# NVlabs/DREAM

Measured on AMD Instinct MI355X. Metric: frames/s DREAM-vgg-q 400x400 b=128 inference, higher is better.
Workload: dtype f32

## Files before the change

dream_amd/csrc/conv_wino4.hip:

```cpp
#include <type_traits>
#include <stdlib.h>
#include <dream_cdna4.h>
#include "common.h"
#include "pack_device.h"
#include "../../include/dream_hip.h"

#ifndef DREAM_W4_DIAG
#define DREAM_W4_DIAG 0
#endif
#ifndef DREAM_W4_STORE
#define DREAM_W4_STORE buffer_store_f32
#endif
#ifndef DREAM_W4_MIDBARRIER
#define DREAM_W4_MIDBARRIER 0
#endif
#ifndef DREAM_W4_STAGGER_N
#define DREAM_W4_STAGGER_N 0
#define DREAM_W4_STAGGER_PCT 0
#endif
#ifndef DREAM_W4_WAUX
#define DREAM_W4_WAUX 0
#endif
#ifndef DREAM_W4_XAUX
#define DREAM_W4_XAUX 0
#endif
#ifndef DREAM_W4_STAG_LX
#define DREAM_W4_STAG_LX 0
#endif
#ifndef DREAM_W4_RUNNING_WOFF
#define DREAM_W4_RUNNING_WOFF 1
#endif
#ifndef DREAM_W4_SETPRIO
#define DREAM_W4_SETPRIO 0
#endif

namespace {

struct Wino4Params {
    const float *x;
    const float *u;
    const float *scale;
    const float *shift;
    const float *residual;
    float *y;
    float *y_full;
    int B, H, W, Cin, Cout, CoutPad;
    int TY, TX;
    int ntiles;
    int nblk, blk_per_xcd;
    unsigned long long magic_tpi, magic_tx;
    int flags;
    int out_scale, out_oy, out_ox;
    int in_scale, in_oy, in_ox;
    int stagger_n, stagger_unit;
    int ymap;
};

constexpr int W4T = 16;
constexpr int W4P = 36;
#ifndef DREAM_W4_RING
#define DREAM_W4_RING 8
#endif
#ifndef DREAM_W4_NARROW_RING
#define DREAM_W4_NARROW_RING 18
#endif
#ifndef DREAM_W4_PAT_RING
#define DREAM_W4_PAT_RING 10
#endif
#ifndef DREAM_W4_PAT_S1OFF
#define DREAM_W4_PAT_S1OFF 8
#endif


template <bool NARROW>
struct W4Cfg {
    static constexpr int NW = NARROW ? 4 : 8;
    static constexpr int K = NARROW ? 8 : 16;
    static constexpr int Q = K / 4;
    static constexpr int KS = K / 4;
    static constexpr int PAD = 16 * NW;
    static constexpr int VPS = NARROW ? W4T * K : W4T * K + 16;
    static constexpr int VB = W4P * VPS;
    static constexpr int SROW = NARROW ? 14 : 25;
    static constexpr int QS = NARROW ? 7 : 6;
    static constexpr int SB = W4T * 6 * SROW * 4;
    static constexpr int RING = NARROW ? DREAM_W4_NARROW_RING : DREAM_W4_RING;
    static constexpr int AHEAD = RING - 2;
    static_assert(72 % RING == 0, "the weight ring must divide two chunks' positions");
    using vec = std::conditional_t<NARROW, f32x2, f32x4>;
};
template <bool NARROW>
DREAM_DEVICE int v4_slot(int q, int t) { return NARROW ? q ^ ((t >> 3) & 1) : q ^ ((t >> 2) & 2); }

DREAM_DEVICE f32x4 fma4(float c, f32x4 a, f32x4 b) {
    f32x4 r;
#pragma unroll
    for (int k = 0; k < 4; ++k) r[k] = __builtin_fmaf(c, a[k], b[k]);
    return r;
}

DREAM_DEVICE f32x4 sub4(f32x4 y, f32x4 x) { return pk_sub4(y, x); }
DREAM_DEVICE f32x4 bt_row(int j, const f32x4 *d) {
    switch (j) {
        case 0: return fma4(-2.0f, d[2], fma4(1.5f, sub4(d[3], d[1]), d[0] + d[4]));
        case 1: return fma4(2.5f, d[3], fma4(0.5f, d[2], sub4(d[4], d[1])));
        case 2: return fma4(0.5f, d[3], fma4(-2.5f, d[2], d[4] + d[1]));
        case 3: return fma4(2.0f, sub4(d[3], d[1]), sub4(d[4], d[2]));
        case 4: return fma4(-0.5f, sub4(d[3], d[1]), sub4(d[4], d[2]));
        default: return fma4(-2.0f, d[3], fma4(1.5f, sub4(d[4], d[2]), d[1] + d[5]));
    }
}

DREAM_DEVICE constexpr bool pat4_row_active(int pat, int i) { return pat == 0 || (((pat - 1) >> 1) == 0 ? i <= 4 : i >= 1); }
DREAM_DEVICE constexpr bool pat4_col_active(int pat, int j) { return pat == 0 || (((pat - 1) & 1) == 0 ? j <= 4 : j >= 1); }
DREAM_DEVICE constexpr bool pat4_active(int pat, int pp) { return pat4_row_active(pat, pp / 6) && pat4_col_active(pat, pp % 6); }
DREAM_DEVICE constexpr int pat4_count(int pat) { return pat == 0 ? 36 : 25; }
struct Pat4Table { int pos[36]; };
constexpr Pat4Table pat4_table(int pat) {
    Pat4Table t = {};
    int n = 0;
    for (int pp = 0; pp < 36; ++pp)
        if (pat4_active(pat, pp)) t.pos[n++] = pp;
    return t;
}
template <int PAT>
struct Pat4 { static constexpr Pat4Table table = pat4_table(PAT); };
#define pat4_pos(PAT, k) (Pat4<PAT>::table.pos[k])

template <int MODE, bool NARROW, int PAT = 0>
__global__ void __launch_bounds__(64 * W4Cfg<NARROW>::NW, 2) conv_wino4_kernel(const Wino4Params p) {
    using C = W4Cfg<NARROW>;
    using vec = typename C::vec;
    constexpr int W4K = C::K, W4NW = C::NW, V4PS = C::VPS, V4B = C::VB, S4ROW = C::SROW;
    constexpr int NPOS = pat4_count(PAT);
    constexpr int W4_RING = PAT ? DREAM_W4_PAT_RING : C::RING, W4_AHEAD = W4_RING - 2;
    static_assert((2 * NPOS) % W4_RING == 0, "the weight ring must divide two chunks' positions");
    DREAM_DYNAMIC_LDS(float, sV);
    const int tid = threadIdx.x;
    const int lane = tid & 63;
    const int wave = wave_index();
    const int item_id = wave * 48 + (lane < 48 ? lane : lane - 16);

    const int xcd = (int)(blockIdx.x & 7), J = (int)(gridDim.x >> 3);
    const int part = p.ymap ? xcd / p.ymap : xcd;
    const int blk_hi = (part + 1) * p.blk_per_xcd;
    const int blk_end = blk_hi < p.nblk ? blk_hi : p.nblk;
    int tb = part * p.blk_per_xcd + (int)(blockIdx.x >> 3);
    if (tb >= blk_end) return;
    const int n0 = (p.ymap ? xcd % p.ymap : (int)blockIdx.y) * (16 * W4NW);
    if (p.stagger_n > 1) {
        const unsigned w = blockIdx.x + blockIdx.y * gridDim.x;
        const int naps = (int)((w * 2654435761u >> 16) % (unsigned)p.stagger_n) * p.stagger_unit;
        for (int i = 0; i < naps; ++i) __builtin_amdgcn_s_sleep(127);
    }
    const int tiles_per_img = p.TY * p.TX;
    const int Si = PAT ? p.in_scale : 1;
    const size_t img_floats = (size_t)(Si * p.H) * (Si * p.W) * p.Cin;

    const int q1 = item_id % C::Q, r1 = (item_id / C::Q) % 6, t1 = (item_id / C::Q) / 6;
    const int s1_off = ((t1 * 6 + r1) * S4ROW + C::QS * q1) * 4;
    const int q2 = item_id % C::Q;
    const int j2 = NARROW ? (item_id >> 3) % 6 : (item_id >> 2) % 6;
    const int t2 = NARROW ? 4 * (item_id / 48) + ((item_id >> 1) & 3) : (item_id >> 2) / 6;
    const int s2_off = ((t2 * 6) * S4ROW + C::QS * q2 + j2) * 4;
    const int v2_off = j2 * V4PS + t2 * W4K + 4 * v4_slot<NARROW>(q2, t2);

    unsigned goff0;
    int item1 = t1 | (r1 << 8) | (q1 << 16);
    auto plan_item = [&](int tile0, int b0) {
        asm volatile("" : "+v"(item1));
        const int t = item1 & 255, r = (item1 >> 8) & 255, q = (item1 >> 16) & 255;
        const int tau = tile0 + t;
        const bool tv = tau < p.ntiles;
        const int b = div_magic40(tau, p.magic_tpi), rem = tau - b * tiles_per_img;
        const int ty = div_magic40(rem, p.magic_tx), tx = rem - ty * p.TX;
        const int gy = 4 * ty - 1 + r, x0 = 4 * tx - 1;
        const bool rok = tv & ((unsigned)gy < (unsigned)p.H);
        goff0 = PAT ? (unsigned)(((((b - b0) * Si * p.H + Si * gy + p.in_oy) * (Si * p.W) + Si * x0 + p.in_ox) * p.Cin + 4 * q) * 4)
                    : (unsigned)(((((b - b0) * p.H + gy) * p.W + x0) * p.Cin + 4 * q) * 4);
        item1 &= 0xffffff;
#pragma unroll
        for (int c = 0; c < 6; ++c) item1 |= (rok & ((unsigned)(x0 + c) < (unsigned)p.W)) ? (1 << (24 + c)) : 0;
    };
    const unsigned px_in = (unsigned)(Si * p.Cin * 4);
    auto item_offset = [&](int c) {
        if (DREAM_W4_DIAG & 16) {
            unsigned o = BUFFER_OOB;
            asm volatile("" : "+v"(o));
            return o;
        }
        return (item1 >> (24 + c)) & 1 ? goff0 + (unsigned)c * px_in : BUFFER_OOB;
    };
    auto block_tile0 = [&](int blk) { return blk < blk_end ? blk * W4T : p.ntiles; };
    auto block_xbuf = [&](int b0) {
        return make_buffer(p.x + (size_t)b0 * img_floats, ((size_t)(p.B - b0) * img_floats) * sizeof(float));
    };

    const int lt = lane & 15, lg = lane >> 4;
    const int a_off = NARROW ? lt * W4K + 4 * v4_slot<NARROW>(lg >> 1, lt) + 2 * (lg & 1) : lt * W4K + 4 * v4_slot<NARROW>(lg, lt);
    const unsigned b_lane = (unsigned)(((wave * 16 + lt) * W4K + C::KS * lg) * 4);
    const unsigned u_pos_stride = (unsigned)(p.CoutPad * W4K * 4);
    const BufferRsrc ubuf = make_buffer(p.u + (size_t)n0 * W4K, ((size_t)((p.Cin / W4K) * W4P + C::AHEAD) * p.CoutPad - (size_t)n0) * W4K * sizeof(float));

    f32x4 acc[W4P];
    const int nchunks = p.Cin / W4K;
    if (DREAM_W4_SETPRIO && wave >= W4NW / 2) __builtin_amdgcn_s_setprio(1);

    vec bq[W4_RING];
    auto load_u = [&](unsigned soff) {
        if constexpr (NARROW) return buffer_load_x2(ubuf, b_lane, soff);
        else return buffer_load_x4_aux<DREAM_W4_WAUX>(ubuf, b_lane, soff);
    };
#pragma unroll
    for (int k = 0; k < W4_AHEAD; ++k) bq[k] = load_u((unsigned)pat4_pos(PAT, k) * u_pos_stride);
    unsigned woff = (unsigned)W4_AHEAD * u_pos_stride;
    DREAM_OPAQUE_SGPR(woff);

    f32x4 *const sV4 = (f32x4 *)sV;
    vec *const sVa = (vec *)sV;
    int vrd[2], vwr[2], s1p = (2 * V4B + s1_off) / 4, s2p = (2 * V4B + s2_off) / 4;
#pragma unroll
    for (int h = 0; h < 2; ++h) {
        vrd[h] = (h * V4B + a_off) / C::KS;
        vwr[h] = (h * V4B + v2_off) / 4;
        asm volatile("" : "+v"(vrd[h]), "+v"(vwr[h]));
    }
    asm volatile("" : "+v"(s1p), "+v"(s2p));
    f32x4 d[6];
    auto pass1_piece = [&](int j) { sV4[s1p + j] = bt_row(j, d); };
    auto pass2_read = [&](int r) { d[r] = sV4[s2p + r * S4ROW]; };
    auto pass2_piece = [&](int i, int h) { if (pat4_row_active(PAT, i)) sV4[vwr[h] + i * (6 * V4PS / 4)] = bt_row(i, d); };

    vec a[2][2];
    auto read_a = [&](int set, int k, int h) {
        const int p0 = pat4_pos(PAT, k), p1 = pat4_pos(PAT, k + 1 < NPOS ? k + 1 : k);
        if constexpr (NARROW) {
            a[set][0] = lds_read_unmerged(sVa + vrd[h] + p0 * V4PS / C::KS);
            a[set][1] = lds_read_unmerged(sVa + vrd[h] + p1 * V4PS / C::KS);
        } else {
            a[set][0] = sVa[vrd[h] + p0 * V4PS / C::KS];
            if (k + 1 < NPOS) a[set][1] = sVa[vrd[h] + p1 * V4PS / C::KS];
        }
    };

    int tile0 = block_tile0(tb);
    int b0 = div_magic40(tile0, p.magic_tpi);
    BufferRsrc xbuf = block_xbuf(b0);
    plan_item(tile0, b0);
#pragma unroll
    for (int c = 0; c < 6; ++c) d[c] = buffer_load_x4(xbuf, item_offset(c), 0u);
#pragma unroll
    for (int j = 0; j < 6; ++j) pass1_piece(j);
    __syncthreads();
#pragma unroll
    for (int r = 0; r < 6; ++r) pass2_read(r);
#pragma unroll
    for (int i = 0; i < 6; ++i) pass2_piece(i, 0);
    __syncthreads();

    auto chunk = [&](auto ph_tag, auto stag_tag, bool last, int c, int tile0n, int b0n) __attribute__((always_inline)) {
        constexpr int PH = decltype(ph_tag)::value;
        constexpr int STAG = decltype(stag_tag)::value;
#ifndef DREAM_W4_S1
#define DREAM_W4_S1 10
#define DREAM_W4_S2 13
#define DREAM_W4_LX 3
#endif
        constexpr int NSLOT = (NPOS + 1) / 2;
        constexpr int S1 = PAT ? NSLOT - DREAM_W4_PAT_S1OFF : DREAM_W4_S1, S2 = PAT ? S1 + 3 : DREAM_W4_S2;
        constexpr int LX = PAT ? 1 : DREAM_W4_LX;
        constexpr int LX0 = STAG ? DREAM_W4_STAG_LX : 0;
        static_assert(LX0 + LX <= S1, "the patch loads must be issued before pass 1");
        const unsigned coff = last ? 0u : (unsigned)((c + 1) * W4K * 4);
        const int cnext = last ? 0 : (c + 1) * W4P;
        if (PH == 1 && last) xbuf = block_xbuf(b0n);
        read_a(0, 0, PH);
        __builtin_amdgcn_sched_barrier(0);
#pragma unroll
        for (int s = 0; s < NSLOT; ++s) {
            const int k0 = 2 * s;
            const bool two = k0 + 1 < NPOS;
            const int pp = pat4_pos(PAT, k0), pp1 = pat4_pos(PAT, two ? k0 + 1 : k0);
            auto load_b = [&](int half) {
                if ((DREAM_W4_DIAG & 2) || (half && !two)) return;
                const int kn = k0 + half + W4_AHEAD;
                if constexpr (PAT == 0 && DREAM_W4_RUNNING_WOFF && !(DREAM_W4_DIAG & 32)) {
                    if (kn == NPOS && last) woff = 0u;
                    bq[(PH * NPOS + kn) % W4_RING] = load_u(woff);
                    woff += u_pos_stride;
                    DREAM_OPAQUE_SGPR(woff);
                } else {
                    const int spos = kn >= NPOS ? cnext + pat4_pos(PAT, kn - NPOS) : c * W4P + pat4_pos(PAT, kn);
                    bq[(PH * NPOS + kn) % W4_RING] = load_u((DREAM_W4_DIAG & 32) ? 0u : (unsigned)spos * u_pos_stride);
                }
            };
            auto load_x = [&](int col) { if (!(DREAM_W4_DIAG & 1)) d[col] = buffer_load_x4_aux<DREAM_W4_XAUX>(xbuf, item_offset(col), (DREAM_W4_DIAG & 64) ? 0u : coff); };
            auto pair = [&](int r) {
                const int i0 = (PH * NPOS + k0) % W4_RING, i1 = (PH * NPOS + k0 + 1) % W4_RING;
                acc[pp] = mfma_f32_16x16x4(a[s & 1][0][r], bq[i0][r], acc[pp]);
                if (two) acc[pp1] = mfma_f32_16x16x4(a[s & 1][1][r], bq[i1][r], acc[pp1]);
                __builtin_amdgcn_sched_barrier(0);
            };
            auto after = [&](int k) {
                if (k == 0) {
                    load_b(0);
                    if (s + 1 < NSLOT) read_a((s + 1) & 1, k0 + 2, PH);
                    if (PH == 1 && s == 0 && last) plan_item(tile0n, b0n);
                    if (s >= LX0 && s < LX0 + LX) { for (int c2 = 0; c2 < 3 / LX; ++c2) load_x((6 / LX) * (s - LX0) + c2); }
                    if (!(DREAM_W4_DIAG & 8) && s >= S1 && s < S1 + 3) pass1_piece(2 * (s - S1));
                    if (!(DREAM_W4_DIAG & 8) && s == S2) { pass2_read(0); pass2_read(1); }
                    if (!(DREAM_W4_DIAG & 8) && s > S2 && s <= S2 + 3) pass2_piece(2 * (s - S2 - 1), 1 - PH);
                } else if (k == 1) {
                    load_b(1);
                    if (s >= LX0 && s < LX0 + LX) { for (int c2 = 3 / LX; c2 < 6 / LX; ++c2) load_x((6 / LX) * (s - LX0) + c2); }
                    if (!(DREAM_W4_DIAG & 8) && s == S2) { pass2_read(2); pass2_read(3); }
                } else if (k == 2) {
                    if (!(DREAM_W4_DIAG & 8) && s >= S1 && s < S1 + 3) pass1_piece(2 * (s - S1) + 1);
                    if (!(DREAM_W4_DIAG & 8) && s == S2) { pass2_read(4); pass2_read(5); }
                    if (!(DREAM_W4_DIAG & 8) && s > S2 && s <= S2 + 3) pass2_piece(2 * (s - S2 - 1) + 1, 1 - PH);
                }
            };
            if constexpr (NARROW) {
                pair(0);
                after(0);
                after(1);
                pair(1);
                after(2);
            } else {
                pair(0);
                after(0);
                pair(1);
                after(1);
                pair(2);
                after(2);
                pair(3);
            }
            if (s == S1 + 2 && !(DREAM_W4_DIAG & 4)) {
                if (DREAM_W4_MIDBARRIER) __syncthreads();
                __builtin_amdgcn_sched_barrier(0);
            }
        }
        if (!(DREAM_W4_DIAG & 4)) __syncthreads();
    };
    const std::integral_constant<int, 0> ph0{};
    const std::integral_constant<int, 1> ph1{};

    constexpr bool pool = MODE == 1 || MODE == 4, both = MODE == 4, has_res = MODE == 2 || MODE == 3, mask = MODE == 3;
    auto epilogue = [&](auto site_tag, int tile0e, int b0e) {
        if (DREAM_W4_DIAG & 128) {
#pragma unroll
            for (int pp = 0; pp < W4P; ++pp)
                if (pat4_active(PAT, pp)) asm volatile("" :: "v"(acc[pp]));
            return;
        }
        const auto &e = *DREAM_KERNARG_SITE(p, decltype(site_tag)::value);
        const bool relu = (e.flags & DREAM_CONV_RELU) != 0;
        const bool late = MODE == 2 && (e.flags & DREAM_CONV_RES_AFTER_RELU) != 0;
        const int Ho = pool ? e.H / 2 : e.H, Wo = pool ? e.W / 2 : e.W, So = e.out_scale;
        const size_t out_img = (size_t)(So * Ho) * (So * Wo) * e.Cout;
        const unsigned px_b = (unsigned)(So * e.Cout * 4), row_b = (unsigned)(So * So * Wo * e.Cout * 4);
        const int ln = lane_id();
        const int lt = ln & 15, lg = ln >> 4;
        const int col = n0 + wave * 16 + lt;
        const bool cok = col < e.Cout;
        const float sc = (e.scale != nullptr && cok) ? e.scale[col] : 1.0f;
        const float sh = (e.shift != nullptr && cok) ? e.shift[col] : 0.0f;
        const BufferRsrc ybuf = make_buffer(e.y + (size_t)b0e * out_img, (DREAM_W4_DIAG & 256) ? 0 : (size_t)(e.B - b0e) * out_img * sizeof(float));
        const BufferRsrc rbuf = make_buffer(has_res ? e.residual + (size_t)b0e * out_img : e.y,
                                            has_res ? (size_t)(e.B - b0e) * out_img * sizeof(float) : 0);
        const size_t full_img = (size_t)e.H * e.W * e.Cout;
        const unsigned fpx_b = (unsigned)(e.Cout * 4), frow_b = (unsigned)(e.W * e.Cout * 4);
        const BufferRsrc fbuf = make_buffer(both ? e.y_full + (size_t)b0e * full_img : e.y, both ? (size_t)(e.B - b0e) * full_img * sizeof(float) : 0);
        const int tau0 = tile0e + lg * 4;
        int b = div_magic40(tau0, p.magic_tpi);
        const int rem = tau0 - b * tiles_per_img;
        int ty = div_magic40(rem, p.magic_tx), tx = rem - ty * p.TX;
        constexpr int NS = pool ? 2 : 4;
        unsigned basef[2][2];
        int limf[2][2];
        unsigned base4[2][2];
        int lim4[2][2];
        constexpr int FULL = pool ? 0x33 : 0xff;
#pragma unroll
        for (int rp = 0; rp < 2; ++rp)
#pragma unroll
            for (int h = 0; h < 2; ++h) {
                const bool tok = cok & ((tau0 + 2 * rp + h) < p.ntiles);
                const int oy = NS * ty, ox = NS * tx;
                base4[rp][h] = (unsigned)(((((b - b0e) * So * Ho + So * oy + e.out_oy) * (So * Wo) + So * ox + e.out_ox) * e.Cout + col) * 4);
                int m = 0;
#pragma unroll
                for (int i = 0; i < NS; ++i) m |= ((oy + i) < Ho ? 1 << i : 0) | ((ox + i) < Wo ? 16 << i : 0);
                lim4[rp][h] = tok ? m : 0;
                if (both) {
                    basef[rp][h] = (unsigned)(((((b - b0e) * e.H + 4 * ty) * e.W + 4 * tx) * e.Cout + col) * 4);
                    int mf = 0;
#pragma unroll
                    for (int i = 0; i < 4; ++i) mf |= ((4 * ty + i) < e.H ? 1 << i : 0) | ((4 * tx + i) < e.W ? 16 << i : 0);
                    limf[rp][h] = tok ? mf : 0;
                }
                const bool wrap_x = (tx + 1 == p.TX);
                const bool wrap_y = wrap_x & (ty + 1 == p.TY);
                tx = wrap_x ? 0 : tx + 1;
                ty = wrap_y ? 0 : (wrap_x ? ty + 1 : ty);
                b += wrap_y ? 1 : 0;
            }
        auto out_off4 = [&](int rp, int h, int i, int jj) {
            const bool inb = ((lim4[rp][h] >> i) & (lim4[rp][h] >> (4 + jj)) & 1) != 0;
            return inb ? base4[rp][h] + (unsigned)i * row_b + (unsigned)jj * px_b : BUFFER_OOB;
        };
        bool interior4[2];
#pragma unroll
        for (int rp = 0; rp < 2; ++rp) interior4[rp] = wave_all((lim4[rp][0] == FULL) & (lim4[rp][1] == FULL));
        auto load_col0 = [&](int rp, float (&r)[2][4]) {
            if (interior4[rp]) {
#pragma unroll
                for (int h = 0; h < 2; ++h)
#pragma unroll
                    for (int i = 0; i < 4; ++i) r[h][i] = buffer_load_f32(rbuf, base4[rp][h], (unsigned)i * row_b);
            } else {
#pragma unroll
                for (int h = 0; h < 2; ++h)
#pragma unroll
                    for (int i = 0; i < 4; ++i) r[h][i] = buffer_load_f32(rbuf, out_off4(rp, h, i, 0), 0u);
            }
        };
        float r0[2][4], r0n[2][4];
        if (has_res) load_col0(0, r0);
#pragma unroll
        for (int rp = 0; rp < 2; ++rp) {
            const unsigned (&base)[2] = base4[rp];
            auto out_off = [&](int h, int i, int jj) { return out_off4(rp, h, i, jj); };
            const bool all_interior = interior4[rp];
            auto fm = [](float c, f32x2 x, f32x2 y) { return __builtin_elementwise_fma(f32x2{c, c}, x, y); };
            f32x2 sA[6][4];
#pragma unroll
            for (int i = 0; i < 6; ++i) {
                f32x2 m[6];
#pragma unroll
                for (int j = 0; j < 6; ++j)
                    m[j] = pat4_active(PAT, 6 * i + j) ? f32x2{acc[6 * i + j][2 * rp], acc[6 * i + j][2 * rp + 1]} : f32x2{0.0f, 0.0f};
                const f32x2 t1 = pk_sub2(m[1], m[2]), t2 = m[1] + m[2];
                sA[i][0] = (m[0] + t2) + (m[3] + m[4]);
                sA[i][1] = fm(-2.0f, m[4], fm(0.5f, m[3], t1));
                sA[i][2] = fm(4.0f, m[4], fm(0.25f, m[3], t2));
                sA[i][3] = fm(-8.0f, m[4], fm(0.125f, m[3], t1)) + m[5];
            }
            auto finish = [&](float v, float rv) {
                if (has_res) v = mask ? (rv > 0.0f ? v : 0.0f) : (late ? v : v + rv);
                const float vr = fmaxf(v, 0.0f);
                v = relu ? vr : v;
                return (MODE == 2 && late) ? v + rv : v;
            };
            auto columns = [&](auto interior_tag, auto &rcur) {
                constexpr bool interior = decltype(interior_tag)::value;
                auto voff = [&](int h, int i, int j2) { return interior ? base[h] : out_off(h, i, j2); };
                auto soff = [&](int i, int j2) { return interior ? (unsigned)i * row_b + (unsigned)j2 * px_b : 0u; };
                float keep[2][2];
#pragma unroll
                for (int jj = 0; jj < 4; ++jj) {
                    float rnext[2][4];
                    if (has_res && jj == 3 && rp == 0) load_col0(1, r0n);
                    if (has_res && jj + 1 < 4) {
#pragma unroll
                        for (int h = 0; h < 2; ++h)
#pragma unroll
                            for (int i = 0; i < 4; ++i) rnext[h][i] = buffer_load_f32(rbuf, voff(h, i, jj + 1), soff(i, jj + 1));
                    }
                    const f32x2 t1 = pk_sub2(sA[1][jj], sA[2][jj]), t2 = sA[1][jj] + sA[2][jj];
                    f32x2 o4[4];
                    o4[0] = (sA[0][jj] + t2) + (sA[3][jj] + sA[4][jj]);
                    o4[1] = fm(-2.0f, sA[4][jj], fm(0.5f, sA[3][jj], t1));
                    o4[2] = fm(4.0f, sA[4][jj], fm(0.25f, sA[3][jj], t2));
                    o4[3] = fm(-8.0f, sA[4][jj], fm(0.125f, sA[3][jj], t1)) + sA[5][jj];
#pragma unroll
                    for (int i = 0; i < 4; ++i) o4[i] = o4[i] * f32x2{sc, sc} + f32x2{sh, sh};
#pragma unroll
                    for (int h = 0; h < 2; ++h) {
                        if (pool) {
                            float v[4];
#pragma unroll
                            for (int i = 0; i < 4; ++i) v[i] = finish(o4[i][h], 0.0f);
                            if (both) {
#pragma unroll
                                for (int i = 0; i < 4; ++i) {
                                    const bool inb = ((limf[rp][h] >> i) & (limf[rp][h] >> (4 + jj)) & 1) != 0;
                                    DREAM_W4_STORE(fbuf, v[i], inb ? basef[rp][h] + (unsigned)i * frow_b + (unsigned)jj * fpx_b : BUFFER_OOB, 0u);
                                }
                            }
                            if ((jj & 1) == 0) {
                                keep[h][0] = fmaxf(v[0], v[1]);
                                keep[h][1] = fmaxf(v[2], v[3]);
                            } else {
                                DREAM_W4_STORE(ybuf, fmaxf(keep[h][0], fmaxf(v[0], v[1])), voff(h, 0, jj >> 1), soff(0, jj >> 1));
                                DREAM_W4_STORE(ybuf, fmaxf(keep[h][1], fmaxf(v[2], v[3])), voff(h, 1, jj >> 1), soff(1, jj >> 1));
                            }
                        } else {
#pragma unroll
                            for (int i = 0; i < 4; ++i)
                                DREAM_W4_STORE(ybuf, finish(o4[i][h], has_res ? rcur[h][i] : 0.0f), voff(h, i, jj), soff(i, jj));
                        }
                    }
                    if (has_res && jj + 1 < 4) {
#pragma unroll
                        for (int h = 0; h < 2; ++h)
#pragma unroll
                            for (int i = 0; i < 4; ++i) rcur[h][i] = rnext[h][i];
                    }
                }
            };
            if (all_interior) columns(std::true_type{}, r0);
            else columns(std::false_type{}, r0);
            if (has_res && rp == 0) {
#pragma unroll
                for (int h = 0; h < 2; ++h)
#pragma unroll
                    for (int i = 0; i < 4; ++i) r0[h][i] = r0n[h][i];
            }
        }
    };

    auto run_blocks = [&](auto stag_tag) __attribute__((always_inline)) {
        while (true) {
            const int tile0n = block_tile0(tb + J);
            const int b0n = div_magic40(tile0n, p.magic_tpi);
            const f32x4 zero = {0.0f, 0.0f, 0.0f, 0.0f};
#pragma unroll
            for (int pp = 0; pp < W4P; ++pp)
                if (pat4_active(PAT, pp)) acc[pp] = zero;
            for (int c = 0; c < nchunks; c += 2) {
                chunk(ph0, stag_tag, false, c, tile0n, b0n);
                chunk(ph1, stag_tag, c + 2 == nchunks, c + 1, tile0n, b0n);
            }
            epilogue(stag_tag, tile0, b0);
            tb += J;
            if (tb >= blk_end) break;
            tile0 = tile0n;
            b0 = b0n;
        }
    };
    if constexpr (!NARROW && PAT == 0 && DREAM_W4_STAG_LX > 0) {
        if (wave >= W4NW / 2) run_blocks(std::integral_constant<int, 1>{});
        else run_blocks(std::integral_constant<int, 0>{});
    } else {
        run_blocks(std::integral_constant<int, 0>{});
    }
}

static_assert(W4Cfg<false>::K == 16 && W4Cfg<false>::PAD == 128 && W4Cfg<true>::K == 8 && W4Cfg<true>::PAD == 64 && W4P == 36,
              "pack_device.h assumes 16-channel chunks padded to 128 rows / 8-channel chunks padded to 64 rows, 36 positions");
__global__ void __launch_bounds__(256) wino4_pack_kernel(const float *w, float *u, int Cout, int Cin, int mode) {
    dream_pack::winograd4(w, u, Cout, Cin, mode, (int)blockIdx.x, (int)gridDim.x);
}

int g_max_workgroups4 = 0;
int g_stagger_n4 = -1, g_stagger_pct4 = 0;
int g_ymap4 = -1;

bool narrow_rows(int rows) { return rows <= W4Cfg<true>::PAD; }
struct PackShape { int k, rows_pad, ahead; };
PackShape pack_shape(int rows) {
    if (narrow_rows(rows)) return {W4Cfg<true>::K, W4Cfg<true>::PAD, W4Cfg<true>::AHEAD};
    return {W4Cfg<false>::K, (rows + W4Cfg<false>::PAD - 1) / W4Cfg<false>::PAD * W4Cfg<false>::PAD, W4Cfg<false>::AHEAD};
}

template <int MODE, bool NARROW, int PAT = 0>
int launch_wino4(const Wino4Params &p, void *stream) {
    using C = W4Cfg<NARROW>;
    void (*kernel)(const Wino4Params) = conv_wino4_kernel<MODE, NARROW, PAT>;
    const size_t lds = ((size_t)2 * C::VB + C::SB) * sizeof(float);
    if (dream_allow_full_lds((const void *)kernel)) return 2;
    const int ny = (p.Cout + 16 * C::NW - 1) / (16 * C::NW);
    const int resident = g_max_workgroups4 > 0 ? g_max_workgroups4 : (NARROW ? 512 : 256);
    Wino4Params q = p;
    dim3 grid;
    if (g_ymap4 && !NARROW && (ny == 2 || ny == 4) && resident >= 64 && p.nblk >= resident) {
        q.ymap = ny;
        q.blk_per_xcd = (p.nblk + 8 / ny - 1) / (8 / ny);
        grid = dim3((unsigned)(resident / 8 * 8), 1u);
    } else {
        int gx = resident / ny / 8 * 8;
        if (gx < 8) gx = 8;
        if (gx > (p.nblk + 7) / 8 * 8) gx = (p.nblk + 7) / 8 * 8;
        grid = dim3((unsigned)gx, (unsigned)ny);
    }
    hipLaunchKernelGGL(kernel, grid, dim3(64 * C::NW), lds, (hipStream_t)stream, q);
    DREAM_LAUNCH_OK();
    return 0;
}

template <bool NARROW>
int launch_wino4_mode(const Wino4Params &p, int mode, void *stream) {
    switch (mode) {
        case 0: return launch_wino4<0, NARROW>(p, stream);
        case 1: return launch_wino4<1, NARROW>(p, stream);
        case 2: return launch_wino4<2, NARROW>(p, stream);
        case 4: return launch_wino4<4, NARROW>(p, stream);
        default: return launch_wino4<3, NARROW>(p, stream);
    }
}

}

extern "C" size_t dream_conv3x3_winograd4_weight_floats(int rows, int cols) {
    const PackShape ps = pack_shape(rows);
    return ((size_t)(cols / ps.k) * W4P + ps.ahead) * ps.rows_pad * ps.k;
}

extern "C" int dream_conv3x3_winograd4_set_channel_block_pinning(int on) {
    DREAM_REQUIRE(on >= -1 && on <= 1, "winograd F(4x4): pinning %d", on);
    g_ymap4 = on;
    return 0;
}

extern "C" int dream_conv3x3_winograd4_set_stagger(int phases, int percent) {
    DREAM_REQUIRE(phases <= 1024 && percent >= 0 && percent <= 400, "winograd F(4x4): stagger %d phases over %d %%", phases, percent);
    g_stagger_n4 = phases < 0 ? -1 : (phases > 1 ? phases : 0);
    g_stagger_pct4 = percent;
    return 0;
}

extern "C" int dream_conv3x3_winograd4_set_max_workgroups(int n) {
    DREAM_REQUIRE(n >= 0, "winograd F(4x4): max workgroups %d", n);
    g_max_workgroups4 = n;
    return 0;
}

extern "C" int dream_pack_conv3x3_winograd4_weight(const float *w_oihw, float *u, int Cout, int Cin, int mode, void *stream) {
    DREAM_REQUIRE(w_oihw && u && Cout > 0 && Cin > 0 && (mode == 0 || mode == 1), "winograd F(4x4) pack: bad arguments");
    const int rows = mode == 0 ? Cout : Cin, cols = mode == 0 ? Cin : Cout;
    const PackShape ps = pack_shape(rows);
    DREAM_REQUIRE(cols % (2 * ps.k) == 0, "winograd F(4x4) pack: %d input channels, must be a multiple of %d", cols, 2 * ps.k);
    const size_t total = (size_t)(cols / ps.k) * ps.rows_pad * ps.k;
    size_t grid = (total + 255) / 256;
    if (grid > 4096) grid = 4096;
    hipLaunchKernelGGL(wino4_pack_kernel, dim3((unsigned)grid), dim3(256), 0, (hipStream_t)stream, w_oihw, u, Cout, Cin, mode);
    DREAM_LAUNCH_OK();
    if (dream_zero_words(u + (size_t)(cols / ps.k) * W4P * ps.rows_pad * ps.k, (size_t)ps.ahead * ps.rows_pad * ps.k * sizeof(float), (hipStream_t)stream))
        return 2;
    return 0;
}

namespace {

int wino4_setup(Wino4Params &p, const float *x, const float *u_packed, const float *scale, const float *shift, const float *residual,
                float *y, int B, int H, int W, int Cin, int Cout, int flags, int out_scale, int in_scale = 1) {
    DREAM_REQUIRE(x && u_packed && y, "winograd F(4x4) conv: null pointer");
    DREAM_REQUIRE(B > 0 && H > 0 && W > 0 && Cin > 0 && Cout > 0, "winograd F(4x4) conv: bad shape B=%d H=%d W=%d Cin=%d Cout=%d", B, H, W, Cin, Cout);
    const PackShape ps = pack_shape(Cout);
    DREAM_REQUIRE(Cin % (2 * ps.k) == 0, "winograd F(4x4) conv: Cin=%d must be a multiple of %d", Cin, 2 * ps.k);
    const size_t span_imgs = (size_t)W4T / ((size_t)((H + 3) / 4) * ((W + 3) / 4)) + 2;
    DREAM_REQUIRE(span_imgs * in_scale * in_scale * H * W * (size_t)Cin * sizeof(float) < ((size_t)1 << 31) &&
                  span_imgs * out_scale * out_scale * H * W * (size_t)Cout * sizeof(float) < ((size_t)1 << 31),
                  "winograd F(4x4) conv: image too large for 32-bit offsets");
    p.x = x; p.u = u_packed; p.scale = scale; p.shift = shift; p.residual = residual; p.y = y; p.y_full = nullptr;
    p.B = B; p.H = H; p.W = W; p.Cin = Cin; p.Cout = Cout;
    p.CoutPad = Cout <= ps.rows_pad ? ps.rows_pad : (Cout + ps.rows_pad - 1) / ps.rows_pad * ps.rows_pad;
    DREAM_REQUIRE(((size_t)(Cin / ps.k) * W4P + ps.ahead) * (size_t)p.CoutPad * ps.k * sizeof(float) < ((size_t)1 << 31), "winograd F(4x4) conv: weights too large");
    p.TY = (H + 3) / 4; p.TX = (W + 3) / 4;
    const long ntiles = (long)B * p.TY * p.TX;
    DREAM_REQUIRE(ntiles < ((long)1 << 24), "winograd F(4x4) conv: %ld tiles, the tile decomposition handles < 2^24", ntiles);
    p.ntiles = (int)ntiles;
    p.nblk = (p.ntiles + W4T - 1) / W4T;
    p.blk_per_xcd = (p.nblk + 7) / 8;
    p.magic_tpi = (((unsigned long long)1 << 40) + (unsigned long long)(p.TY * p.TX) - 1) / (unsigned long long)(p.TY * p.TX);
    p.magic_tx = (((unsigned long long)1 << 40) + (unsigned long long)p.TX - 1) / (unsigned long long)p.TX;
    p.flags = flags;
    p.out_scale = out_scale; p.out_oy = 0; p.out_ox = 0;
    p.in_scale = in_scale; p.in_oy = 0; p.in_ox = 0;
    p.ymap = 0;
    if (g_stagger_n4 < 0) {
        const char *e = getenv("DREAM_W4_STAGGER");
        int n = DREAM_W4_STAGGER_N, pct = DREAM_W4_STAGGER_PCT;
        if (e != nullptr && sscanf(e, "%d,%d", &n, &pct) != 2) { n = DREAM_W4_STAGGER_N; pct = DREAM_W4_STAGGER_PCT; }
        g_stagger_n4 = n > 1 ? n : 0;
        g_stagger_pct4 = pct;
    }
    {
        const double chunk_cycles = narrow_rows(Cout) ? 7000.0 : 13500.0;
        const double block_naps = (double)(Cin / ps.k) * chunk_cycles / 8128.0;
        p.stagger_n = g_stagger_n4;
        p.stagger_unit = g_stagger_n4 > 1 ? (int)(block_naps * g_stagger_pct4 / 100.0 / g_stagger_n4 + 0.5) : 0;
        if (p.stagger_n > 1 && p.stagger_unit < 1) p.stagger_unit = 1;
    }
    if (g_ymap4 < 0) {
        const char *e = getenv("DREAM_W4_YMAP");
        g_ymap4 = (e != nullptr && e[0] == '0') ? 0 : 1;
    }
    return 0;
}

}

extern "C" int dream_conv3x3_winograd4_nhwc_f32(const float *x, const float *u_packed, const float *scale, const float *shift,
                                                const float *residual, float *y, int B, int H, int W, int Cin, int Cout, int flags,
                                                void *stream) {
    DREAM_REQUIRE((flags & ~(DREAM_CONV_RELU | DREAM_CONV_POOL2 | DREAM_CONV_RELUMASK | DREAM_CONV_RES_AFTER_RELU)) == 0, "winograd F(4x4) conv: unsupported flags 0x%x", flags);
    DREAM_REQUIRE(!(flags & DREAM_CONV_RES_AFTER_RELU) || (residual != nullptr && !(flags & (DREAM_CONV_POOL2 | DREAM_CONV_RELUMASK))),
                  "winograd F(4x4) conv: residual-after-ReLU needs a residual and excludes the fused pool / the ReLU mask");
    DREAM_REQUIRE(!(flags & DREAM_CONV_POOL2) || (residual == nullptr && H >= 2 && W >= 2), "winograd F(4x4) conv: fused max-pool takes no residual");
    DREAM_REQUIRE(!(flags & DREAM_CONV_RELUMASK) || residual != nullptr, "winograd F(4x4) conv: ReLU mask without a mask tensor");
    Wino4Params p;
    if (int rc = wino4_setup(p, x, u_packed, scale, shift, residual, y, B, H, W, Cin, Cout, flags, 1)) return rc;
    const int mode = (flags & DREAM_CONV_POOL2) ? 1 : (flags & DREAM_CONV_RELUMASK) ? 3 : (residual != nullptr ? 2 : 0);
    return narrow_rows(Cout) ? launch_wino4_mode<true>(p, mode, stream) : launch_wino4_mode<false>(p, mode, stream);
}

extern "C" int dream_conv3x3_winograd4_pool_both_nhwc_f32(const float *x, const float *u_packed, const float *scale, const float *shift,
                                                          float *y_full, float *y_pool, int B, int H, int W, int Cin, int Cout, int flags,
                                                          void *stream) {
    DREAM_REQUIRE((flags & ~DREAM_CONV_RELU) == 0, "winograd F(4x4) conv + pool: unsupported flags 0x%x", flags);
    DREAM_REQUIRE(y_full != nullptr && y_pool != nullptr && H >= 2 && W >= 2, "winograd F(4x4) conv + pool: null output or map too small");
    Wino4Params p;
    if (int rc = wino4_setup(p, x, u_packed, scale, shift, nullptr, y_pool, B, H, W, Cin, Cout, flags, 1)) return rc;
    p.y_full = y_full;
    return narrow_rows(Cout) ? launch_wino4_mode<true>(p, 4, stream) : launch_wino4_mode<false>(p, 4, stream);
}

extern "C" size_t dream_convT4x4_winograd4_weight_floats(int Cout, int Cin) { return 4 * dream_conv3x3_winograd4_weight_floats(Cout, Cin); }

extern "C" int dream_pack_convT4x4_winograd4_weight(const float *wT, float *u4, float *scratch, int Cin, int Cout, int mode, void *stream) {
    DREAM_REQUIRE(wT && u4 && scratch && Cin > 0 && Cout > 0 && (mode == 0 || mode == 1), "winograd F(4x4) convT pack: bad arguments");
    if (int rc = dream_convT4x4_phase_weights(wT, scratch, Cin, Cout, mode, stream)) return rc;
    const int rows = mode == 0 ? Cout : Cin, cols = mode == 0 ? Cin : Cout;
    const size_t per_u = dream_conv3x3_winograd4_weight_floats(rows, cols);
    for (int ph = 0; ph < 4; ++ph)
        if (int rc = dream_pack_conv3x3_winograd4_weight(scratch + (size_t)ph * Cout * Cin * 9, u4 + ph * per_u, rows, cols, 0, stream)) return rc;
    return 0;
}

extern "C" int dream_conv4x4s2_winograd4_nhwc_f32(const float *dy, const float *u4, float *dx, int B, int H, int W, int Cout, int Cin,
                                                  void *stream) {
    DREAM_REQUIRE(Cin > 64, "winograd F(4x4) conv4x4s2: needs more than 64 output channels (the wide workgroup shape), got %d", Cin);
    Wino4Params p;
    if (int rc = wino4_setup(p, dy, u4, nullptr, nullptr, nullptr, dx, B, H, W, Cout, Cin, 0, 1, 2)) return rc;
    const size_t per_u = dream_conv3x3_winograd4_weight_floats(Cin, Cout);
    for (int ph = 0; ph < 4; ++ph) {
        p.u = u4 + ph * per_u;
        p.in_oy = ph >> 1; p.in_ox = ph & 1;
        p.residual = ph == 0 ? nullptr : dx;
        int rc;
        switch (ph) {
            case 0: rc = launch_wino4<0, false, 4>(p, stream); break;
            case 1: rc = launch_wino4<2, false, 3>(p, stream); break;
            case 2: rc = launch_wino4<2, false, 2>(p, stream); break;
            default: rc = launch_wino4<2, false, 1>(p, stream); break;
        }
        if (rc) return rc;
    }
    return 0;
}

extern "C" int dream_conv_transpose4x4s2_winograd4_nhwc_f32(const float *x, const float *u4, const float *scale, const float *shift,
                                                            float *y, int B, int H, int W, int Cin, int Cout, int flags, void *stream) {
    DREAM_REQUIRE((flags & ~DREAM_CONV_RELU) == 0, "winograd F(4x4) convT: unsupported flags 0x%x", flags);
    DREAM_REQUIRE(Cout > 64, "winograd F(4x4) convT: needs more than 64 output channels (the wide workgroup shape), got %d", Cout);
    Wino4Params p;
    if (int rc = wino4_setup(p, x, u4, scale, shift, nullptr, y, B, H, W, Cin, Cout, flags, 2)) return rc;
    const size_t per_u = dream_conv3x3_winograd4_weight_floats(Cout, Cin);
    for (int ph = 0; ph < 4; ++ph) {
        p.u = u4 + ph * per_u;
        p.out_oy = ph >> 1; p.out_ox = ph & 1;
        int rc;
        switch (ph) {
            case 0: rc = launch_wino4<0, false, 1>(p, stream); break;
            case 1: rc = launch_wino4<0, false, 2>(p, stream); break;
            case 2: rc = launch_wino4<0, false, 3>(p, stream); break;
            default: rc = launch_wino4<0, false, 4>(p, stream); break;
        }
        if (rc) return rc;
    }
    return 0;
}
```

Baseline: 2569.

## Overlap Winograd output epilogue of previous block with next block's first chunk

For the default pattern and the plain and pooled modes, the output transform and stores of the previous tile block are now interleaved into the first input-channel chunk of the next block instead of running as a separate serial epilogue. The first chunk visits transform positions in a permuted order (columns 4-5 first, then columns 0-3), so accumulators are consumed by the epilogue before MFMAs overwrite them with a zero init. The weight-offset walk is reworked to follow that permutation. The aim is to hide epilogue ALU and store latency behind MFMA work, at the cost of more register pressure, a more intricate schedule and a fragile weight-offset sequence.

Measured after the change: 2563. Within noise of the previous version (-0.2%).

```diff
diff --git a/dream_amd/csrc/conv_wino4.hip b/dream_amd/csrc/conv_wino4.hip
--- a/dream_amd/csrc/conv_wino4.hip
+++ b/dream_amd/csrc/conv_wino4.hip
@@ -32,6 +32,12 @@
 #endif
 #ifndef DREAM_W4_SETPRIO
 #define DREAM_W4_SETPRIO 0
+#endif
+#ifndef DREAM_W4_STRAIGHT_EPILOGUE
+#define DREAM_W4_STRAIGHT_EPILOGUE 0
+#endif
+#ifndef DREAM_W4_MERGE_LX0
+#define DREAM_W4_MERGE_LX0 0
 #endif
 
 namespace {
@@ -127,6 +133,19 @@
 struct Pat4 { static constexpr Pat4Table table = pat4_table(PAT); };
 #define pat4_pos(PAT, k) (Pat4<PAT>::table.pos[k])
 
+struct Perm4Table { int pos[36]; };
+constexpr Perm4Table perm4_table() {
+    Perm4Table t = {};
+    int n = 0;
+    for (int i = 0; i < 6; ++i)
+        for (int j = 4; j < 6; ++j) t.pos[n++] = 6 * i + j;
+    for (int j = 0; j < 4; ++j)
+        for (int i = 0; i < 6; ++i) t.pos[n++] = 6 * i + j;
+    return t;
+}
+struct Perm4 { static constexpr Perm4Table table = perm4_table(); };
+#define perm4_pos(k) (Perm4::table.pos[k])
+
 template <int MODE, bool NARROW, int PAT = 0>
 __global__ void __launch_bounds__(64 * W4Cfg<NARROW>::NW, 2) conv_wino4_kernel(const Wino4Params p) {
     using C = W4Cfg<NARROW>;
@@ -135,6 +154,7 @@
     constexpr int NPOS = pat4_count(PAT);
     constexpr int W4_RING = PAT ? DREAM_W4_PAT_RING : C::RING, W4_AHEAD = W4_RING - 2;
     static_assert((2 * NPOS) % W4_RING == 0, "the weight ring must divide two chunks' positions");
+    constexpr bool OVERLAP = !DREAM_W4_STRAIGHT_EPILOGUE && !(DREAM_W4_DIAG & (32 | 128 | 256)) && DREAM_W4_RUNNING_WOFF && PAT == 0 && (MODE == 0 || MODE == 1);
     DREAM_DYNAMIC_LDS(float, sV);
     const int tid = threadIdx.x;
     const int lane = tid & 63;
@@ -212,8 +232,8 @@
         else return buffer_load_x4_aux<DREAM_W4_WAUX>(ubuf, b_lane, soff);
     };
 #pragma unroll
-    for (int k = 0; k < W4_AHEAD; ++k) bq[k] = load_u((unsigned)pat4_pos(PAT, k) * u_pos_stride);
-    unsigned woff = (unsigned)W4_AHEAD * u_pos_stride;
+    for (int k = 0; k < W4_AHEAD; ++k) bq[k] = load_u((unsigned)(OVERLAP ? perm4_pos(k) : pat4_pos(PAT, k)) * u_pos_stride);
+    unsigned woff = (unsigned)(OVERLAP ? perm4_pos(W4_AHEAD) : W4_AHEAD) * u_pos_stride;
     DREAM_OPAQUE_SGPR(woff);
 
     f32x4 *const sV4 = (f32x4 *)sV;
@@ -232,8 +252,9 @@
     auto pass2_piece = [&](int i, int h) { if (pat4_row_active(PAT, i)) sV4[vwr[h] + i * (6 * V4PS / 4)] = bt_row(i, d); };
 
     vec a[2][2];
-    auto read_a = [&](int set, int k, int h) {
-        const int p0 = pat4_pos(PAT, k), p1 = pat4_pos(PAT, k + 1 < NPOS ? k + 1 : k);
+    auto read_a = [&](int set, int k, int h, bool merged = false) {
+        const int k1 = k + 1 < NPOS ? k + 1 : k;
+        const int p0 = merged ? perm4_pos(k) : pat4_pos(PAT, k), p1 = merged ? perm4_pos(k1) : pat4_pos(PAT, k1);
         if constexpr (NARROW) {
             a[set][0] = lds_read_unmerged(sVa + vrd[h] + p0 * V4PS / C::KS);
             a[set][1] = lds_read_unmerged(sVa + vrd[h] + p1 * V4PS / C::KS);
@@ -258,9 +279,124 @@
     for (int i = 0; i < 6; ++i) pass2_piece(i, 0);
     __syncthreads();
 
-    auto chunk = [&](auto ph_tag, auto stag_tag, bool last, int c, int tile0n, int b0n) __attribute__((always_inline)) {
+    constexpr bool pool = MODE == 1 || MODE == 4, both = MODE == 4, has_res = MODE == 2 || MODE == 3, mask = MODE == 3;
+    f32x2 sA2[2][6][4];
+    f32x2 eo[4];
+    unsigned ebase[2][2], epx_b, erow_b;
+    int elim;
+    int eflags, steady = 0;
+    float esc, esh, ekeep[2][2][2];
+    BufferRsrc eybuf;
+    auto fm2 = [](float c, f32x2 x, f32x2 y) { return __builtin_elementwise_fma(f32x2{c, c}, x, y); };
+    auto pin2 = [](f32x2 &v) {
+        float v0 = v[0], v1 = v[1];
+        asm volatile("" : "+v"(v0), "+v"(v1));
+        v = f32x2{v0, v1};
+    };
+    auto epi_rows = [&](int tile0e, int b0e) {
+        const auto &e = *DREAM_KERNARG_SITE(p, 2);
+        eflags = (e.flags & DREAM_CONV_RELU) != 0 ? 1 : 0;
+        const int Ho = pool ? e.H / 2 : e.H, Wo = pool ? e.W / 2 : e.W;
+        const size_t out_img = (size_t)Ho * Wo * e.Cout;
+        epx_b = (unsigned)(e.Cout * 4);
+        erow_b = (unsigned)(Wo * e.Cout * 4);
+        int bl = (int)(b_lane >> 2);
+        asm volatile("" : "+v"(bl));
+        const int lt = (bl / W4K) & 15, lg = (bl % W4K) / C::KS;
+        const int col = n0 + wave * 16 + lt;
+        const bool cok = col < e.Cout;
+        esc = (e.scale != nullptr && cok) ? e.scale[col] : 1.0f;
+        esh = (e.shift != nullptr && cok) ? e.shift[col] : 0.0f;
+        eybuf = make_buffer(e.y + (size_t)b0e * out_img, steady ? (size_t)(e.B - b0e) * out_img * sizeof(float) : 0);
+#pragma unroll
+        for (int i = 0; i < 6; ++i)
+#pragma unroll
+            for (int rp = 0; rp < 2; ++rp) {
+                f32x2 m[6];
+#pragma unroll
+                for (int j = 0; j < 6; ++j) m[j] = f32x2{acc[6 * i + j][2 * rp], acc[6 * i + j][2 * rp + 1]};
+                const f32x2 t1 = pk_sub2(m[1], m[2]), t2 = m[1] + m[2];
+                sA2[rp][i][0] = (m[0] + t2) + (m[3] + m[4]);
+                sA2[rp][i][1] = fm2(-2.0f, m[4], fm2(0.5f, m[3], t1));
+                sA2[rp][i][2] = fm2(4.0f, m[4], fm2(0.25f, m[3], t2));
+                sA2[rp][i][3] = fm2(-8.0f, m[4], fm2(0.125f, m[3], t1)) + m[5];
+#pragma unroll
+                for (int jj = 0; jj < 4; ++jj) pin2(sA2[rp][i][jj]);
+                __builtin_amdgcn_sched_barrier(0);
+            }
+        const int tau0 = tile0e + lg * 4;
+        int b = div_magic40(tau0, p.magic_tpi);
+        const int rem = tau0 - b * tiles_per_img;
+        int ty = div_magic40(rem, p.magic_tx), tx = rem - ty * p.TX;
+        constexpr int NS = pool ? 2 : 4, FULL = pool ? 0x33 : 0xff;
+#pragma unroll
+        for (int rp = 0; rp < 2; ++rp) {
+#pragma unroll
+            for (int h = 0; h < 2; ++h) {
+                const bool tok = cok & ((tau0 + 2 * rp + h) < p.ntiles);
+                const int oy = NS * ty, ox = NS * tx;
+                ebase[rp][h] = (unsigned)(((((b - b0e) * Ho + oy) * Wo + ox) * e.Cout + col) * 4);
+                int m = 0;
+#pragma unroll
+                for (int i = 0; i < NS; ++i) m |= ((oy + i) < Ho ? 1 << i : 0) | ((ox + i) < Wo ? 16 << i : 0);
+                elim = (rp == 0 && h == 0 ? 0 : elim) | ((tok ? m : 0) << (8 * (2 * rp + h)));
+                const bool wrap_x = (tx + 1 == p.TX);
+                const bool wrap_y = wrap_x & (ty + 1 == p.TY);
+                tx = wrap_x ? 0 : tx + 1;
+                ty = wrap_y ? 0 : (wrap_x ? ty + 1 : ty);
+                b += wrap_y ? 1 : 0;
+            }
+            eflags |= wave_all(((elim >> (16 * rp)) & 0xffff) == (FULL | FULL << 8)) ? 2 << rp : 0;
+        }
+    };
+    auto epi_column = [&](int rp, int jj) {
+        const f32x2 (&s)[6][4] = sA2[rp];
+        const f32x2 t1 = pk_sub2(s[1][jj], s[2][jj]), t2 = s[1][jj] + s[2][jj];
+        eo[0] = (s[0][jj] + t2) + (s[3][jj] + s[4][jj]);
+        eo[1] = fm2(-2.0f, s[4][jj], fm2(0.5f, s[3][jj], t1));
+        eo[2] = fm2(4.0f, s[4][jj], fm2(0.25f, s[3][jj], t2));
+        eo[3] = fm2(-8.0f, s[4][jj], fm2(0.125f, s[3][jj], t1)) + s[5][jj];
+#pragma unroll
+        for (int i = 0; i < 4; ++i) {
+            eo[i] = eo[i] * f32x2{esc, esc} + f32x2{esh, esh};
+            pin2(eo[i]);
+        }
+    };
+    auto epi_store = [&](int rp, int jj, int h) {
+        float v[4];
+#pragma unroll
+        for (int i = 0; i < 4; ++i) {
+            const float vr = fmaxf(eo[i][h], 0.0f);
+            v[i] = (eflags & 1) ? vr : eo[i][h];
+        }
+        auto off = [&](int i, int j2) {
+            const bool inb = ((elim >> (8 * (2 * rp + h) + i)) & (elim >> (8 * (2 * rp + h) + 4 + j2)) & 1) != 0;
+            return inb ? ebase[rp][h] + (unsigned)i * erow_b + (unsigned)j2 * epx_b : BUFFER_OOB;
+        };
+        if (pool) {
+            if ((jj & 1) == 0) {
+                ekeep[rp][h][0] = fmaxf(v[0], v[1]);
+                ekeep[rp][h][1] = fmaxf(v[2], v[3]);
+                return;
+            }
+            v[0] = fmaxf(ekeep[rp][h][0], fmaxf(v[0], v[1]));
+            v[1] = fmaxf(ekeep[rp][h][1], fmaxf(v[2], v[3]));
+        }
+        const int j2 = pool ? jj >> 1 : jj;
+        if (eflags & (2 << rp)) {
+#pragma unroll
+            for (int i = 0; i < (pool ? 2 : 4); ++i) DREAM_W4_STORE(eybuf, v[i], ebase[rp][h], (unsigned)i * erow_b + (unsigned)j2 * epx_b);
+        } else {
+#pragma unroll
+            for (int i = 0; i < (pool ? 2 : 4); ++i) DREAM_W4_STORE(eybuf, v[i], off(i, j2), 0u);
+        }
+    };
+
+    auto chunk = [&](auto ph_tag, auto stag_tag, auto merged_tag, bool last, int c, int tile0n, int b0n) __attribute__((always_inline)) {
         constexpr int PH = decltype(ph_tag)::value;
         constexpr int STAG = decltype(stag_tag)::value;
+        constexpr bool MERGED = decltype(merged_tag)::value;
+        static_assert(!MERGED || (PH == 0 && OVERLAP), "the merged body is chunk 0 of a block");
 #ifndef DREAM_W4_S1
 #define DREAM_W4_S1 10
 #define DREAM_W4_S2 13
@@ -269,22 +405,37 @@
         constexpr int NSLOT = (NPOS + 1) / 2;
         constexpr int S1 = PAT ? NSLOT - DREAM_W4_PAT_S1OFF : DREAM_W4_S1, S2 = PAT ? S1 + 3 : DREAM_W4_S2;
         constexpr int LX = PAT ? 1 : DREAM_W4_LX;
-        constexpr int LX0 = STAG ? DREAM_W4_STAG_LX : 0;
+        constexpr int LX0 = MERGED ? DREAM_W4_MERGE_LX0 : STAG ? DREAM_W4_STAG_LX : 0;
         static_assert(LX0 + LX <= S1, "the patch loads must be issued before pass 1");
         const unsigned coff = last ? 0u : (unsigned)((c + 1) * W4K * 4);
         const int cnext = last ? 0 : (c + 1) * W4P;
         if (PH == 1 && last) xbuf = block_xbuf(b0n);
-        read_a(0, 0, PH);
+        if constexpr (MERGED) {
+            const int tile0e = steady ? (tb - J) * W4T : 0;
+            epi_rows(tile0e, div_magic40(tile0e, p.magic_tpi));
+            __builtin_amdgcn_sched_barrier(0);
+        }
+        const f32x4 zero = {0.0f, 0.0f, 0.0f, 0.0f};
+        read_a(0, 0, PH, MERGED);
         __builtin_amdgcn_sched_barrier(0);
 #pragma unroll
         for (int s = 0; s < NSLOT; ++s) {
             const int k0 = 2 * s;
             const bool two = k0 + 1 < NPOS;
-            const int pp = pat4_pos(PAT, k0), pp1 = pat4_pos(PAT, two ? k0 + 1 : k0);
+            const int pp = MERGED ? perm4_pos(k0) : pat4_pos(PAT, k0), pp1 = MERGED ? perm4_pos(k0 + 1) : pat4_pos(PAT, two ? k0 + 1 : k0);
             auto load_b = [&](int half) {
                 if ((DREAM_W4_DIAG & 2) || (half && !two)) return;
                 const int kn = k0 + half + W4_AHEAD;
-                if constexpr (PAT == 0 && DREAM_W4_RUNNING_WOFF && !(DREAM_W4_DIAG & 32)) {
+                if constexpr (OVERLAP) {
+                    if (MERGED && kn == NPOS) woff = (unsigned)W4P * u_pos_stride;
+                    if (PH == 1 && kn == NPOS && last) woff = (unsigned)perm4_pos(0) * u_pos_stride;
+                    bq[(PH * NPOS + kn) % W4_RING] = load_u(woff);
+                    const int kq = MERGED ? kn : kn - NPOS;
+                    const unsigned dperm = kq >= 0 && kq + 1 < NPOS ? (unsigned)(perm4_pos(kq + 1) - perm4_pos(kq)) : 1u;
+                    if (MERGED) woff += (kn < NPOS ? dperm : 1u) * u_pos_stride;
+                    else woff += (PH == 1 && kn >= NPOS && last ? dperm : 1u) * u_pos_stride;
+                    DREAM_OPAQUE_SGPR(woff);
+                } else if constexpr (PAT == 0 && DREAM_W4_RUNNING_WOFF && !(DREAM_W4_DIAG & 32)) {
                     if (kn == NPOS && last) woff = 0u;
                     bq[(PH * NPOS + kn) % W4_RING] = load_u(woff);
                     woff += u_pos_stride;
@@ -297,14 +448,18 @@
             auto load_x = [&](int col) { if (!(DREAM_W4_DIAG & 1)) d[col] = buffer_load_x4_aux<DREAM_W4_XAUX>(xbuf, item_offset(col), (DREAM_W4_DIAG & 64) ? 0u : coff); };
             auto pair = [&](int r) {
                 const int i0 = (PH * NPOS + k0) % W4_RING, i1 = (PH * NPOS + k0 + 1) % W4_RING;
-                acc[pp] = mfma_f32_16x16x4(a[s & 1][0][r], bq[i0][r], acc[pp]);
-                if (two) acc[pp1] = mfma_f32_16x16x4(a[s & 1][1][r], bq[i1][r], acc[pp1]);
+                acc[pp] = mfma_f32_16x16x4(a[s & 1][0][r], bq[i0][r], MERGED && r == 0 ? zero : acc[pp]);
+                if (two) acc[pp1] = mfma_f32_16x16x4(a[s & 1][1][r], bq[i1][r], MERGED && r == 0 ? zero : acc[pp1]);
                 __builtin_amdgcn_sched_barrier(0);
             };
             auto after = [&](int k) {
+                if constexpr (MERGED) {
+                    if (s < 8 && k == 0) epi_column(s & 1, s >> 1);
+                    if (s < 8 && k > 0) epi_store(s & 1, s >> 1, k - 1);
+                }
                 if (k == 0) {
                     load_b(0);
-                    if (s + 1 < NSLOT) read_a((s + 1) & 1, k0 + 2, PH);
+                    if (s + 1 < NSLOT) read_a((s + 1) & 1, k0 + 2, PH, MERGED);
                     if (PH == 1 && s == 0 && last) plan_item(tile0n, b0n);
                     if (s >= LX0 && s < LX0 + LX) { for (int c2 = 0; c2 < 3 / LX; ++c2) load_x((6 / LX) * (s - LX0) + c2); }
                     if (!(DREAM_W4_DIAG & 8) && s >= S1 && s < S1 + 3) pass1_piece(2 * (s - S1));
@@ -323,6 +478,7 @@
             if constexpr (NARROW) {
                 pair(0);
                 after(0);
+                if (MERGED) __builtin_amdgcn_sched_barrier(0);
                 after(1);
                 pair(1);
                 after(2);
@@ -345,7 +501,6 @@
     const std::integral_constant<int, 0> ph0{};
     const std::integral_constant<int, 1> ph1{};
 
-    constexpr bool pool = MODE == 1 || MODE == 4, both = MODE == 4, has_res = MODE == 2 || MODE == 3, mask = MODE == 3;
     auto epilogue = [&](auto site_tag, int tile0e, int b0e) {
         if (DREAM_W4_DIAG & 128) {
 #pragma unroll
@@ -520,7 +675,30 @@
         }
     };
 
+    const std::false_type plain{};
     auto run_blocks = [&](auto stag_tag) __attribute__((always_inline)) {
+        if constexpr (OVERLAP) {
+            const f32x4 zero = {0.0f, 0.0f, 0.0f, 0.0f};
+#pragma unroll
+            for (int pp = 0; pp < W4P; ++pp) acc[pp] = zero;
+            steady = 0;
+            while (true) {
+                const int tile0n = block_tile0(tb + J);
+                const int b0n = div_magic40(tile0n, p.magic_tpi);
+                chunk(ph0, stag_tag, std::true_type{}, false, 0, tile0n, b0n);
+                chunk(ph1, stag_tag, plain, nchunks == 2, 1, tile0n, b0n);
+                for (int c = 2; c < nchunks; c += 2) {
+                    chunk(ph0, stag_tag, plain, false, c, tile0n, b0n);
+                    chunk(ph1, stag_tag, plain, c + 2 == nchunks, c + 1, tile0n, b0n);
+                }
+                tb += J;
+                steady = 1;
+                if (tb >= blk_end) break;
+            }
+            const int tile0e = (tb - J) * W4T;
+            epilogue(stag_tag, tile0e, div_magic40(tile0e, p.magic_tpi));
+            return;
+        }
         while (true) {
             const int tile0n = block_tile0(tb + J);
             const int b0n = div_magic40(tile0n, p.magic_tpi);
@@ -529,8 +707,8 @@
             for (int pp = 0; pp < W4P; ++pp)
                 if (pat4_active(PAT, pp)) acc[pp] = zero;
             for (int c = 0; c < nchunks; c += 2) {
-                chunk(ph0, stag_tag, false, c, tile0n, b0n);
-                chunk(ph1, stag_tag, c + 2 == nchunks, c + 1, tile0n, b0n);
+                chunk(ph0, stag_tag, plain, false, c, tile0n, b0n);
+                chunk(ph1, stag_tag, plain, c + 2 == nchunks, c + 1, tile0n, b0n);
             }
             epilogue(stag_tag, tile0, b0);
             tb += J;
```
